# smartroboticslab/okvis2

Measured on AMD Instinct MI355X. Metric: front-end stereo-frames/s (detect+describe+match), 752x480 stereo, higher is better.
Workload: dtype u8/int32 (detect, describe, Hamming) + f64 (match gate); 1 GPU; EuRoC-shaped 752x480 stereo, euroc.yaml front-end params (radius 38, thr 150, <=700 kpts, match thr 60); lanes_per_gpu=1, score_kernels_serialised_across_lanes=False, stereo_frames_per_launch=3072, distinct_frames=256, content=corners, feed=device, cameras_per_multiframe=2, parallelism=frames sharded over 1 GPU(s), no collective

## Files before the change

okvis2_amd/csrc/k_harris.hip:

```cpp
#include <cstdlib>
#include <type_traits>

#include "okvfe_internal.h"

namespace okvfe {

namespace {

constexpr int kTH = 32;
#ifndef OKVFE_K1_WPB
#define OKVFE_K1_WPB 4
#endif
constexpr int kWavesPerBlock = OKVFE_K1_WPB;

__device__ __forceinline__ int mul24(int a, int b) {
  int d;
  asm("v_mul_i32_i24 %0, %1, %2" : "=v"(d) : "v"(a), "v"(b));
  return d;
}
__device__ __forceinline__ int mad24(int a, int b, int c) {
  int d;
  asm("v_mad_i32_i24 %0, %1, %2, %3" : "=v"(d) : "v"(a), "v"(b), "v"(c));
  return d;
}
__device__ __forceinline__ int mad24_10(int a, int c) {
  int d;
  asm("v_mad_i32_i24 %0, %1, 10, %2" : "=v"(d) : "v"(a), "v"(c));
  return d;
}
__device__ __forceinline__ int mul24_3(int a) {
  int d;
  asm("v_mul_i32_i24 %0, 3, %1" : "=v"(d) : "v"(a));
  return d;
}

template <bool ALIGNED>
__device__ __forceinline__ void load_raw(const uint8_t* __restrict__ img, int w, int h, int row,
                                         int x0, int dl, int dc, int dr, uint32_t raw[3]) {
  row = row < 0 ? 0 : (row > h - 1 ? h - 1 : row);
  if (ALIGNED) {
    const uint32_t* rq = reinterpret_cast<const uint32_t*>(img + (size_t)row * (size_t)w);
    raw[0] = rq[dl];
    raw[1] = rq[dc];
    raw[2] = rq[dr];
  } else {
    const uint8_t* rp = img + (size_t)row * (size_t)w;
    uint32_t lo = 0, hi = 0;
#pragma unroll
    for (int i = 0; i < 4; ++i) {
      int c0 = x0 - 2 + i, c1 = x0 + 2 + i;
      c0 = c0 < 0 ? 0 : (c0 > w - 1 ? w - 1 : c0);
      c1 = c1 < 0 ? 0 : (c1 > w - 1 ? w - 1 : c1);
      lo |= (uint32_t)rp[c0] << (8 * i);
      hi |= (uint32_t)rp[c1] << (8 * i);
    }
    raw[0] = lo;
    raw[1] = hi;
    raw[2] = 0;
  }
}

template <bool ALIGNED>
__device__ __forceinline__ void unpack(const uint32_t raw[3], int p[8]) {
  if (ALIGNED) {
    const uint32_t L = raw[0], C = raw[1], R = raw[2];
    p[0] = (L >> 16) & 255;
    p[1] = (L >> 24);
    p[2] = C & 255;
    p[3] = (C >> 8) & 255;
    p[4] = (C >> 16) & 255;
    p[5] = (C >> 24);
    p[6] = R & 255;
    p[7] = (R >> 8) & 255;
  } else {
#pragma unroll
    for (int i = 0; i < 4; ++i) {
      p[i] = (raw[0] >> (8 * i)) & 255;
      p[4 + i] = (raw[1] >> (8 * i)) & 255;
    }
  }
}

__device__ __forceinline__ void cov_row(const int a[8], const int b[8], const int c[8],
                                        const int cmask[6], int rmask, int hs[3][4]) {
  int vs[8], vd[8];
#pragma unroll
  for (int i = 0; i < 8; ++i) {
    vs[i] = mad24_10(b[i], mul24_3(a[i] + c[i]));
    vd[i] = c[i] - a[i];
  }
  int gxx[6], gyy[6], gxy[6];
#pragma unroll
  for (int i = 0; i < 6; ++i) {
    const int m = cmask[i] & rmask;
    const int gx = (vs[i + 2] - vs[i]) & m;
    const int gy = mad24_10(vd[i + 1], mul24_3(vd[i] + vd[i + 2])) & m;
    gxx[i] = mul24(gx, gx) >> 14;
    gyy[i] = mul24(gy, gy) >> 14;
    gxy[i] = mul24(gx, gy) >> 14;
  }
#pragma unroll
  for (int i = 0; i < 4; ++i) {
    hs[0][i] = gxx[i] + 2 * gxx[i + 1] + gxx[i + 2];
    hs[1][i] = gyy[i] + 2 * gyy[i + 1] + gyy[i + 2];
    hs[2][i] = gxy[i] + 2 * gxy[i + 1] + gxy[i + 2];
  }
}

template <bool ALIGNED>
__global__ __launch_bounds__(64 * kWavesPerBlock) void harris_generic_kernel(
    const uint8_t* __restrict__ images, int w, int h, int32_t* __restrict__ scores) {
  const int lane = threadIdx.x;
  const int x0 = (blockIdx.x * 64 + lane) * 4;
  const int wave = __builtin_amdgcn_readfirstlane(threadIdx.y);
  const int ys = (blockIdx.y * kWavesPerBlock + wave) * kTH;
  if (ys >= h || x0 >= w) return;
  const int ye = ys + kTH < h ? ys + kTH : h;
  const size_t img_off = (size_t)blockIdx.z * (size_t)w * (size_t)h;
  const uint8_t* img = images + img_off;
  int32_t* out = scores + img_off + x0;

  const int nd = w >> 2;
  int dc = x0 >> 2;
  dc = dc > nd - 1 ? nd - 1 : dc;
  const int dl = dc > 0 ? dc - 1 : 0;
  const int dr = dc < nd - 1 ? dc + 1 : nd - 1;
  int cmask[6], smask[4];
#pragma unroll
  for (int i = 0; i < 6; ++i) {
    const int col = x0 - 1 + i;
    cmask[i] = (col >= 1 && col <= w - 2) ? -1 : 0;
  }
#pragma unroll
  for (int i = 0; i < 4; ++i) smask[i] = cmask[i + 1];

  int pr[3][8];
  int hsr[3][3][4];
  uint32_t raw[3][3];
  {
    uint32_t t0[3], t1[3];
    load_raw<ALIGNED>(img, w, h, ys - 2, x0, dl, dc, dr, t0);
    load_raw<ALIGNED>(img, w, h, ys - 1, x0, dl, dc, dr, t1);
    load_raw<ALIGNED>(img, w, h, ys, x0, dl, dc, dr, raw[0]);
    load_raw<ALIGNED>(img, w, h, ys + 1, x0, dl, dc, dr, raw[1]);
    unpack<ALIGNED>(t0, pr[0]);
    unpack<ALIGNED>(t1, pr[1]);
  }

  auto step = [&](int j, int s_new, int s_a, int s_b, int h_new, int h_a, int h_b) {
    const int r = ys + j;
    load_raw<ALIGNED>(img, w, h, r + 2, x0, dl, dc, dr, raw[s_new]);
    unpack<ALIGNED>(raw[s_a], pr[s_new]);
    const int g = r - 1;
    const int rmask = (g >= 1 && g <= h - 2) ? -1 : 0;
    cov_row(pr[s_a], pr[s_b], pr[s_new], cmask, rmask, hsr[h_new]);
    const int y = g - 1;
    if (j >= 2 && y < ye) {
      const int ymask = (y >= 1 && y <= h - 2) ? -1 : 0;
      int sc[4];
#pragma unroll
      for (int i = 0; i < 4; ++i) {
        const int A = hsr[h_a][0][i] + 2 * hsr[h_b][0][i] + hsr[h_new][0][i];
        const int B = hsr[h_a][1][i] + 2 * hsr[h_b][1][i] + hsr[h_new][1][i];
        const int Cc = hsr[h_a][2][i] + 2 * hsr[h_b][2][i] + hsr[h_new][2][i];
        const int tq = ((A >> 1) + (B >> 1)) >> 1;
        const int det = mul24(A, B) - mul24(Cc, Cc);
        sc[i] = (det - mul24(tq, tq)) & (smask[i] & ymask);
      }
      int32_t* op = out + (size_t)y * (size_t)w;
      if (ALIGNED) {
        *reinterpret_cast<int4*>(op) = make_int4(sc[0], sc[1], sc[2], sc[3]);
      } else {
#pragma unroll
        for (int i = 0; i < 4; ++i)
          if (x0 + i < w) op[i] = sc[i];
      }
    }
  };

  const int jn = (ye - ys) + 2;
  for (int j = 0; j < jn; j += 3) {
    step(j, 2, 0, 1, 0, 1, 2);
    if (j + 1 < jn) step(j + 1, 0, 1, 2, 1, 2, 0);
    if (j + 2 < jn) step(j + 2, 1, 2, 0, 2, 0, 1);
  }
}


__device__ __forceinline__ int mulhi24(int a, int b) {
  int d;
  asm("v_mul_hi_i32_i24 %0, %1, %2" : "=v"(d) : "v"(a), "v"(b));
  return d;
}
__device__ __forceinline__ void dpp_fence(int& a, int& b, int& c, int& d, int& e, int& f) {
  asm volatile("s_nop 1" : "+v"(a), "+v"(b), "+v"(c), "+v"(d), "+v"(e), "+v"(f));
}
__device__ __forceinline__ void dpp_fence4(int& a, int& b, int& c, int& d) {
  asm volatile("s_nop 1" : "+v"(a), "+v"(b), "+v"(c), "+v"(d));
}
__device__ __forceinline__ void dpp_fence2(int& a, int& b) {
  asm volatile("s_nop 1" : "+v"(a), "+v"(b));
}
__device__ __forceinline__ void lane_neighbours(int a, int b, int& l, int& r) {
  asm("s_nop 1\n\t"
      "v_mov_b32_dpp %0, %2 wave_shr:1 row_mask:0xf bank_mask:0xf bound_ctrl:1\n\t"
      "v_mov_b32_dpp %1, %3 wave_shl:1 row_mask:0xf bank_mask:0xf bound_ctrl:1"
      : "=&v"(l), "=&v"(r)
      : "v"(a), "v"(b));
}
__device__ __forceinline__ int from_left(int v) {
  return __builtin_amdgcn_update_dpp(0, v, 0x138, 0xf, 0xf, true);
}
__device__ __forceinline__ int from_right(int v) {
  return __builtin_amdgcn_update_dpp(0, v, 0x130, 0xf, 0xf, true);
}

constexpr int kStripLanes = 62;
#ifndef OKVFE_K1_WAVES
#define OKVFE_K1_WAVES __attribute__((amdgpu_waves_per_eu(5, 8)))
#endif

struct NmsOut {
  int thr;
  Candidate* cand;
  int cand_cap;
  int32_t* cand_count;
  int32_t* fix_count;
  int32_t* fix_list;
  int no_map;
};

__device__ __forceinline__ int max3i(int a, int b, int c) { return max(max(a, b), c); }
#ifndef OKVFE_K1_SLOTS
#define OKVFE_K1_SLOTS 8
#endif
constexpr int kScoreSlots = OKVFE_K1_SLOTS;
__device__ __forceinline__ void push_hit(uint64_t& mask, uint64_t& ovf, int c, int nb, uint64_t own, uint32_t tag,
                                         uint32_t& sp, uint32_t sp_end) {
  uint64_t sav, pm;
  uint32_t vtag;
  asm volatile(
      "v_cmp_ge_i32_e64 %[mask], %[c], %[nb]\n\t"
      "s_mov_b64 %[ovf], 0\n\t"
      "s_and_b64 %[pm], %[mask], %[own]\n\t"
      "s_cbranch_scc0 .Lokvfe_nopush%=\n\t"
      "s_and_saveexec_b64 %[sav], %[pm]\n\t"
      "v_cmp_gt_u32_e32 vcc, %[end], %[sp]\n\t"
      "s_andn2_b64 %[ovf], exec, vcc\n\t"
      "s_and_b64 exec, exec, vcc\n\t"
      "v_mov_b32 %[vtag], %[tag]\n\t"
      "ds_write2_b32 %[sp], %[c], %[vtag] offset1:64\n\t"
      "v_add_u32 %[sp], %[stride], %[sp]\n\t"
      "s_mov_b64 exec, %[sav]\n"
      ".Lokvfe_nopush%=:"
      : [sp] "+v"(sp), [mask] "=&s"(mask), [ovf] "=&s"(ovf), [sav] "=&s"(sav), [pm] "=&s"(pm), [vtag] "=&v"(vtag)
      : [c] "v"(c), [nb] "v"(nb), [own] "s"(own), [tag] "s"(tag), [end] "s"(sp_end), [stride] "i"(512)
      : "vcc", "scc", "memory");
}

#ifndef OKVFE_K1_STAGE
#define OKVFE_K1_STAGE 248
#endif
constexpr int kCandStage = OKVFE_K1_STAGE;

template <int kTHF, bool NMS, bool PACK = false, bool MEMONLY = false, bool NOMAP = false>
__global__ __launch_bounds__(64 * kWavesPerBlock) OKVFE_K1_WAVES void harris_kernel(
    const uint8_t* __restrict__ images, int w, int h, int32_t* __restrict__ scores, int pitch, int strips,
    int rtiles, int n_images, NmsOut nms, int pack_g, int pack_u, int main_blocks) {
  constexpr int kMain = NMS ? kTHF - 1 : kTHF;
  static_assert(kMain % 6 == 0 && kTHF <= 121, "rows per wave: 6k (+1 with the fused NMS), <= 121");
  constexpr int kSlots = kTHF > 64 ? kScoreSlots + 2 : kScoreSlots;
  const int lane = threadIdx.x;
  const int nd = w >> 2;
  int image, tile, strip, d;
  int sub = 0;
  int group_images = 1;
  bool lane_on = true;
  const bool packed_block = PACK && (int)blockIdx.x >= main_blocks;
  const int wave = __builtin_amdgcn_readfirstlane(threadIdx.y);
  int row_tile;
  if (packed_block) {
    const int p = ((int)blockIdx.x - main_blocks) * kWavesPerBlock + wave;
    const int group = p / rtiles;
    row_tile = p - group * rtiles;
    image = group * pack_g;
    if (image >= n_images) return;
    group_images = n_images - image < pack_g ? n_images - image : pack_g;
    strip = strips;
    sub = lane / pack_u;
    const int j = lane - sub * pack_u;
    lane_on = sub < group_images;
    if (!lane_on) sub = 0;
    d = lane_on ? strip * kStripLanes + j : nd;
  } else {
    const int T = strips * rtiles;
    const int n8 = n_images & ~7;
    const int S = (n8 >> 3) * T;
    const int full = 8 * ((S + kWavesPerBlock - 1) / kWavesPerBlock);
    const int L = (int)blockIdx.x;
    if (L < full) {
      const int s = (L >> 3) * kWavesPerBlock + wave;
      if (s >= S) return;
      const int g = s / T;
      image = g * 8 + (L & 7);
      tile = s - g * T;
    } else {
      const int r = (L - full) * kWavesPerBlock + wave;
      const int i = r / T;
      if (n8 + i >= n_images) return;
      image = n8 + i;
      tile = r - i * T;
    }
    row_tile = tile / strips;
    strip = tile - row_tile * strips;
    d = strip * kStripLanes + lane;
  }
  const int ys_own = row_tile * kTHF;
  if (ys_own >= h) return;
  const int ye_own = ys_own + kTHF < h ? ys_own + kTHF : h;
  const int ys = NMS ? ys_own - 1 : ys_own;
  const bool last_strip = PACK ? packed_block : strip * kStripLanes + 64 >= nd;
  const bool first_lane_halo = packed_block ? d == strip * kStripLanes : (strip != 0 && lane < 1);
  const bool store = d < nd && !first_lane_halo && (last_strip || lane <= kStripLanes);
  const int dcl = d < nd ? d : nd - 1;
  const size_t img_off = (size_t)image * (size_t)w * (size_t)h;
  const __amdgpu_buffer_rsrc_t img_rsrc = __builtin_amdgcn_make_buffer_rsrc(
      const_cast<uint8_t*>(images + img_off), 0, w * h * group_images, 0x00027000);
  const __amdgpu_buffer_rsrc_t out_rsrc = __builtin_amdgcn_make_buffer_rsrc(
      scores + (size_t)image * (size_t)pitch * (size_t)h, 0, pitch * h * 4 * group_images, 0x00027000);
  const int ld_off = dcl * 4 + (PACK ? sub * w * h : 0);
  const bool slotted = NMS && pitch != w;
  const int slot_q = slotted ? d + 2 * strip : d;
  const bool st_on = slotted ? (lane_on && slot_q * 4 < pitch) : store;
  const int st_off = st_on ? slot_q * 16 + (PACK ? sub * pitch * h * 4 : 0) : 0x7FFFFFF0;
  int m0 = d == 0 ? 0 : -1;
  int m3 = d == nd - 1 ? 0 : -1;
  asm volatile("" : "+v"(m0), "+v"(m3));

  auto unpack4 = [](uint32_t c, int p[4]) {
    p[0] = c & 255;
    p[1] = (c >> 8) & 255;
    p[2] = (c >> 16) & 255;
    p[3] = c >> 24;
  };
  (void)unpack4;
  typedef int v4i_t __attribute__((ext_vector_type(4)));
  int win[3][2];
  auto taps = [](int b0, int b1, int b2, int b3) {
    return (int)((uint32_t)(b0 & 255) | ((uint32_t)(b1 & 255) << 8) | ((uint32_t)(b2 & 255) << 16) |
                 ((uint32_t)(b3 & 255) << 24));
  };
  const int r4 = lane & 3;
  int A_above = r4 == 0 ? taps(-24, 0, 24, 0) : r4 == 1 ? taps(0, -24, 0, 24)
              : r4 == 2 ? taps(-24, -80, -24, 0) : taps(0, -24, -80, -24);
  int A_centre = r4 == 0 ? taps(-80, 0, 80, 0) : r4 == 1 ? taps(0, -80, 0, 80) : 0;
  int A_below = r4 == 0 ? taps(-24, 0, 24, 0) : r4 == 1 ? taps(0, -24, 0, 24)
              : r4 == 2 ? taps(24, 80, 24, 0) : taps(0, 24, 80, 24);
  asm volatile("" : "+v"(A_above), "+v"(A_centre), "+v"(A_below));
  auto make_windows = [&](uint32_t dw, int wn[2]) {
    const int x = (int)(dw ^ 0x80808080u);
    int l, r;
    lane_neighbours(x, x, l, r);
    wn[0] = (int)__builtin_amdgcn_alignbyte((uint32_t)x, (uint32_t)l, 3);
    wn[1] = (int)__builtin_amdgcn_alignbyte((uint32_t)r, (uint32_t)x, 1);
  };
  int hs[2][2][4];
  int vp[2][2][4];
#pragma unroll
  for (int q = 0; q < 2; ++q)
#pragma unroll
    for (int c = 0; c < 2; ++c)
#pragma unroll
      for (int i = 0; i < 4; ++i) hs[q][c][i] = vp[q][c][i] = 0;

  int nc[4] = {0, 0, 0, 0}, nh[2][4] = {{0, 0, 0, 0}, {0, 0, 0, 0}}, nl = 0, nr = 0;
  __shared__ int32_t hit_stack[NMS ? kWavesPerBlock * kSlots * 128 : 1];
  constexpr int kStageCap = kCandStage;
  __shared__ Candidate cand_stage[NMS ? kWavesPerBlock : 1][NMS ? kCandStage : 1];
  const uint32_t sp0 = (uint32_t)(uintptr_t)(__attribute__((address_space(3))) int32_t*)hit_stack +
                       (uint32_t)(wave * (kSlots * 512) + lane * 4);
  uint32_t sp = sp0;
  const uint32_t sp_end = (uint32_t)(uintptr_t)(__attribute__((address_space(3))) int32_t*)hit_stack +
                          (uint32_t)((wave + 1) * (kSlots * 512));
  const uint64_t own_lo = __ballot(store && d != 0);
  const uint64_t own_hi = __ballot(store && d != nd - 1);
  const uint64_t real_lanes = __ballot(d < nd);
  const int r_lo = ys_own > 2 ? ys_own : 2;
  const int r_hi = ye_own < h - 2 ? ye_own : h - 2;
  uint64_t rows_adj[2] = {0ull, 0ull};
  auto emit_overflow = [&](uint64_t ovf, int c, int i, int r, bool flag) {
    if ((ovf >> lane) & 1ull) {
      int sub_o = 0;
      if (packed_block) {
        sub_o = lane / pack_u;
        if (sub_o >= group_images) sub_o = 0;
      }
      const int img = image + sub_o;
      const int p = atomicAdd(&nms.cand_count[img], 1);
      if (p < nms.cand_cap) {
        Candidate cd;
        cd.x = dcl * 4 + i;
        cd.y = flag ? r | kCandidateFixupFlag : r;
        cd.score = c;
        nms.cand[(size_t)img * nms.cand_cap + p] = cd;
      }
      if (flag) {
        const int k = atomicAdd(&nms.fix_count[img], 1);
        if (k < kFixListCap) nms.fix_list[(size_t)img * kFixListCap + k] = p;
      }
    }
  };

  auto cov_row = [&](const int* wa, const int* wb, const int* wc, int (*H)[4], bool inner) {
    v4i_t acc1 = {0, 0, 0, 0}, acc2 = {0, 0, 0, 0};
    acc1 = __builtin_amdgcn_mfma_i32_4x4x4i8(A_above, wa[0], acc1, 0, 0, 0);
    acc2 = __builtin_amdgcn_mfma_i32_4x4x4i8(A_above, wa[1], acc2, 0, 0, 0);
    acc1 = __builtin_amdgcn_mfma_i32_4x4x4i8(A_centre, wb[0], acc1, 0, 0, 0);
    acc2 = __builtin_amdgcn_mfma_i32_4x4x4i8(A_centre, wb[1], acc2, 0, 0, 0);
    acc1 = __builtin_amdgcn_mfma_i32_4x4x4i8(A_below, wc[0], acc1, 0, 0, 0);
    acc2 = __builtin_amdgcn_mfma_i32_4x4x4i8(A_below, wc[1], acc2, 0, 0, 0);
#ifndef OKVFE_K1_MFMA_NOPS
#define OKVFE_K1_MFMA_NOPS 7
#endif
#define OKVFE_STR2(x) #x
#define OKVFE_STR(x) OKVFE_STR2(x)
    asm volatile("s_nop " OKVFE_STR(OKVFE_K1_MFMA_NOPS) : "+v"(acc1), "+v"(acc2));
    asm volatile("" ::"v"(wa[0]), "v"(wa[1]), "v"(wb[0]), "v"(wb[1]), "v"(wc[0]), "v"(wc[1]), "v"(A_above), "v"(A_centre),
                 "v"(A_below));
    if (__builtin_expect(!inner, 0)) {
      asm volatile("" ::: "memory");
      acc1 = v4i_t{0, 0, 0, 0};
      acc2 = v4i_t{0, 0, 0, 0};
    }
    int gx[4], gy[4];
    gx[0] = (acc1[0] << 6) & m0;
    gx[1] = acc1[1] << 6;
    gx[2] = acc2[0] << 6;
    gx[3] = (acc2[1] << 6) & m3;
    gy[0] = (acc1[2] << 6) & m0;
    gy[1] = acc1[3] << 6;
    gy[2] = acc2[2] << 6;
    gy[3] = (acc2[3] << 6) & m3;
    int G[2][4];
#pragma unroll
    for (int i = 0; i < 4; ++i) {
      int g0 = mulhi24(gx[i], gx[i]);
      asm("v_mul_hi_i32_i24_sdwa %0, %1, %1 dst_sel:WORD_1 dst_unused:UNUSED_PRESERVE "
          "src0_sel:DWORD src1_sel:DWORD"
          : "+v"(g0)
          : "v"(gy[i]));
      G[0][i] = g0;
      G[1][i] = mulhi24(gx[i], gy[i]);
    }
    dpp_fence4(G[0][0], G[0][3], G[1][0], G[1][3]);
#pragma unroll
    for (int ch = 0; ch < 2; ++ch) {
      int gl, gr;
      lane_neighbours(G[ch][3], G[ch][0], gl, gr);
      const int pm = gl + G[ch][0];
      const int p0 = G[ch][0] + G[ch][1];
      const int p1 = G[ch][1] + G[ch][2];
      const int p2 = G[ch][2] + G[ch][3];
      const int p3 = G[ch][3] + gr;
      H[ch][0] = pm + p0;
      H[ch][1] = p0 + p1;
      H[ch][2] = p1 + p2;
      H[ch][3] = p2 + p3;
    }
  };
  auto score_row = [&](int (*Vp)[4], int (*V)[4], int sc[4]) {
#pragma unroll
    for (int i = 0; i < 4; ++i) {
      const unsigned AB = (unsigned)(Vp[0][i] + V[0][i]);
      const int Cc = Vp[1][i] + V[1][i];
      const int tq = (int)((((AB >> 1) & 0x7FFFu) + (AB >> 17)) >> 1);
      int ab;
      asm("v_mul_u32_u24_sdwa %0, %1, %1 dst_sel:DWORD dst_unused:UNUSED_PAD src0_sel:WORD_0 "
          "src1_sel:WORD_1"
          : "=v"(ab)
          : "v"(AB));
      sc[i] = ab - mad24(tq, tq, mul24(Cc, Cc));
    }
    sc[0] &= m0;
    sc[3] &= m3;
  };
  const bool store_map = !NOMAP && (MEMONLY || !NMS || nms.no_map == 0);
  auto store_row = [&](const int sc[4], int y) {
    if (!store_map) return;
    typedef int v4i __attribute__((ext_vector_type(4)));
    const v4i v = {sc[0], sc[1], sc[2], sc[3]};
    __builtin_amdgcn_raw_buffer_store_b128(v, out_rsrc, st_off, y * pitch * 4, 0);
#ifndef OKVFE_K1_NO_STORE_NOP
    asm volatile("s_nop 1" ::"v"(v));
#endif
  };
  auto nms_row = [&](const int sc[4], int q, bool test, int r) {
    int l, r2;
    lane_neighbours(sc[3], sc[0], l, r2);
    const int hn[4] = {max3i(l, sc[0], sc[1]), max3i(sc[0], sc[1], sc[2]),
                       max3i(sc[1], sc[2], sc[3]), max3i(sc[2], sc[3], r2)};
#ifndef OKVFE_K1_SKIP
#define OKVFE_K1_SKIP 1
#endif
    if (test && r >= r_lo && r < r_hi &&
        (!OKVFE_K1_SKIP || __builtin_amdgcn_ballot_w64(max(nh[q ^ 1][1], nh[q ^ 1][2]) >= nms.thr) != 0ull)) {
      const int lft[4] = {nl, nc[0], nc[1], nc[2]};
      const int rgt[4] = {nc[1], nc[2], nc[3], nr};
      uint64_t mk[4], ovf[4];
#pragma unroll
      for (int i = 0; i < 4; ++i)
        push_hit(mk[i], ovf[i], nc[i], max3i(max3i(nh[q][i], hn[i], lft[i]), rgt[i], nms.thr), i < 2 ? own_lo : own_hi,
                 (uint32_t)(r << 2 | i), sp, sp_end);
      const uint64_t adj = ((mk[0] & mk[1]) | (mk[1] & mk[2]) | (mk[2] & mk[3]) | (mk[3] & (mk[0] >> 1))) & real_lanes;
      if (adj != 0ull) {
        const int t = r - ys_own;
        if (kTHF <= 64 || t < 64)
          rows_adj[0] |= 1ull << t;
        else
          rows_adj[1] |= 1ull << (t - 64);
      }
      if (__builtin_expect((ovf[0] | ovf[1] | ovf[2] | ovf[3]) != 0ull, 0)) {
#pragma unroll
        for (int i = 0; i < 4; ++i) emit_overflow(ovf[i], nc[i], i, r, adj != 0ull);
      }
    }
#pragma unroll
    for (int i = 0; i < 4; ++i) {
      nh[q][i] = hn[i];
      nc[i] = sc[i];
    }
    nl = l;
    nr = r2;
  };

#ifndef OKVFE_K1_AHEAD
#define OKVFE_K1_AHEAD 3
#endif
  constexpr int kAhead = OKVFE_K1_AHEAD;
  static_assert(kAhead >= 1 && kAhead <= 5, "prefetch distance");
  int row_next = ys - 2;
  auto load_next = [&]() -> uint32_t {
    const int r = row_next < 0 ? 0 : (row_next > h - 1 ? h - 1 : row_next);
    ++row_next;
    return (uint32_t)__builtin_amdgcn_raw_buffer_load_b32(img_rsrc, ld_off, r * w, 0);
  };
  uint32_t ring[6];
  {
    const uint32_t t0 = load_next(), t1 = load_next();
#pragma unroll
    for (int i = 0; i < kAhead; ++i) ring[i] = load_next();
    make_windows(t0, win[0]);
    make_windows(t1, win[1]);
  }
  int y = ys - 2;
  auto step = [&](auto ph, auto want_score, auto want_store, auto want_test) {
    constexpr int PH = decltype(ph)::value;
    constexpr int s_new = (PH + 2) % 3, s_a = PH % 3, s_b = (PH + 1) % 3, q = PH % 2;
    ring[(PH + kAhead) % 6] = load_next();
    const int g = y + 1;
    const bool inner = g >= 1 && g <= h - 2;
    if constexpr (MEMONLY) {
      int sc[4];
      unpack4(ring[PH], sc);
      if (decltype(want_store)::value && y < h) store_row(sc, y);
      ++y;
      (void)inner;
      return;
    }
    make_windows(ring[PH], win[s_new]);
    cov_row(win[s_a], win[s_b], win[s_new], hs[q], inner);
#pragma unroll
    for (int ch = 0; ch < 2; ++ch)
#pragma unroll
      for (int i = 0; i < 4; ++i) vp[q][ch][i] = hs[q ^ 1][ch][i] + hs[q][ch][i];
    if (decltype(want_score)::value) {
      int sc[4];
      score_row(vp[q ^ 1], vp[q], sc);
      if (decltype(want_store)::value) {
        if (y < h) store_row(sc, y);
      }
      if (NMS) nms_row(sc, q, decltype(want_test)::value, y - 1);
    }
    ++y;
  };
  using T = std::true_type;
  using F = std::false_type;
#define OKVFE_PH(n) std::integral_constant<int, (n) % 6>()
  step(OKVFE_PH(0), F(), F(), F());
  step(OKVFE_PH(1), F(), F(), F());
  if (NMS) {
    step(OKVFE_PH(2), T(), F(), F());
    step(OKVFE_PH(3), T(), T(), F());
    for (int g = 0; g < kMain / 6; ++g) {
      step(OKVFE_PH(4), T(), T(), T());
      step(OKVFE_PH(5), T(), T(), T());
      step(OKVFE_PH(6), T(), T(), T());
      step(OKVFE_PH(7), T(), T(), T());
      step(OKVFE_PH(8), T(), T(), T());
      step(OKVFE_PH(9), T(), T(), T());
    }
    step(OKVFE_PH(kTHF + 3), T(), F(), T());
  } else {
    for (int g = 0; g < kMain / 6; ++g) {
      step(OKVFE_PH(2), T(), T(), F());
      step(OKVFE_PH(3), T(), T(), F());
      step(OKVFE_PH(4), T(), T(), F());
      step(OKVFE_PH(5), T(), T(), F());
      step(OKVFE_PH(6), T(), T(), F());
      step(OKVFE_PH(7), T(), T(), F());
    }
  }
#undef OKVFE_PH
  if (ys_own == 0 || ye_own == h) {
    const int zero[4] = {0, 0, 0, 0};
    if (ys_own == 0) store_row(zero, 0);
    if (ye_own == h) store_row(zero, h - 1);
  }

  if (NMS) {
    const int cnt = (int)((sp - sp0) >> 9);
    if (!__any(cnt != 0)) return;
    int sub_e = 0;
    if (packed_block) {
      int l2 = lane;
      asm volatile("" : "+v"(l2));
      sub_e = l2 / pack_u;
      if (sub_e >= group_images) sub_e = 0;
    }
    const int image_l = image + sub_e;
    const int x0 = dcl * 4;
    Candidate* outc = nms.cand + (size_t)image_l * nms.cand_cap;
    const int32_t* mine = hit_stack + wave * (kSlots * 128) + lane;
    auto flag_record = [&](int at) {
      const int k = atomicAdd(&nms.fix_count[image_l], 1);
      if (k < kFixListCap) nms.fix_list[(size_t)image_l * kFixListCap + k] = at;
    };
    auto record = [&](int e, bool* flagged) {
      Candidate cd;
      const int tag = mine[e * 128 + 64];
      cd.score = mine[e * 128];
      cd.x = x0 + (tag & 3);
      cd.y = tag >> 2;
      const int t = cd.y - ys_own;
      const uint64_t bit = (kTHF <= 64 || t < 64) ? rows_adj[0] >> t : rows_adj[1] >> (t - 64);
      *flagged = (bit & 1ull) != 0ull;
      if (*flagged) cd.y |= kCandidateFixupFlag;
      return cd;
    };
    auto scan = [&](int c, int* total) {
      int incl = c;
#pragma unroll
      for (int dd = 1; dd < 64; dd <<= 1) {
        const int t = __shfl_up(incl, dd);
        if (lane >= dd) incl += t;
      }
      *total = __builtin_amdgcn_readlane(incl, 63);
      return incl - c;
    };
    if (packed_block) {
      int pos = 0;
      for (int g = 0; g < group_images; ++g) {
        const bool in_g = sub_e == g;
        if (!__any(in_g && cnt != 0)) continue;
        int total;
        const int first = scan(in_g ? cnt : 0, &total);
        int base = 0;
        if (lane == 0) base = atomicAdd(&nms.cand_count[image + g], total);
        base = __builtin_amdgcn_readlane(base, 0);
        if (in_g) pos = base + first;
      }
      for (int e = 0; __any(e < cnt); ++e)
        if (e < cnt) {
          bool fl;
          const Candidate cd = record(e, &fl);
          if (pos + e < nms.cand_cap) outc[pos + e] = cd;
          if (fl) flag_record(pos + e);
        }
    } else {
      int total;
      const int first = scan(cnt, &total);
      int base_l0 = 0;
      if (lane == 0) base_l0 = atomicAdd(&nms.cand_count[image], total);
      constexpr int cap_stage = kStageCap;
      Candidate* stage = cand_stage[wave];
      for (int e = 0; __any(e < cnt); ++e)
        if (e < cnt) {
          bool fl;
          const Candidate cd = record(e, &fl);
          const int idx = first + e;
          if (idx < cap_stage) {
            stage[idx] = cd;
          } else {
            const int at = __builtin_amdgcn_readlane(base_l0, 0) + idx;
            if (at < nms.cand_cap) outc[at] = cd;
          }
          if (fl) flag_record(__builtin_amdgcn_readlane(base_l0, 0) + idx);
        }
      __builtin_amdgcn_wave_barrier();
      const int base = __builtin_amdgcn_readlane(base_l0, 0);
      const int n_staged = total < cap_stage ? total : cap_stage;
      for (int r = lane; r < n_staged; r += 64)
        if (base + r < nms.cand_cap) outc[base + r] = stage[r];
    }
  }
}

}

static int harris_strips(int w) {
  const int nd = w >> 2;
  int strips = 1;
  while ((strips - 1) * kStripLanes + 64 < nd) ++strips;
  return strips;
}

ScoreLayout harris_nms_layout(int w, int h) {
  (void)h;
  static const bool off = lab_env("OKVFE_NO_FUSED_NMS") != nullptr;
  if (off || w % 4 != 0) return ScoreLayout{w, 0};
  const int strips = harris_strips(w);
  if (strips == 1) return ScoreLayout{w, 1};
  const int pitch = ((w + 8 * (strips - 1)) + 31) & ~31;
  return ScoreLayout{pitch, strips};
}

static bool launch_harris_impl(const uint8_t* img, int w, int h, int n_images, int32_t* score,
                               ScoreLayout layout, const NmsOut* nms, hipStream_t stream, bool byte_mover = false) {
  if (n_images <= 0) return true;
  const dim3 block(64, kWavesPerBlock, 1);
  const bool aligned = (w % 4 == 0) && ((reinterpret_cast<uintptr_t>(img) & 3) == 0) &&
                       ((reinterpret_cast<uintptr_t>(score) & 15) == 0);
  if (aligned) {
    const int nd = w >> 2;
    const int strips = harris_strips(w);
    if (nms && !(layout.strips == strips || (layout.strips == 1 && layout.pitch == w))) return false;
    static const int th_env = [] {
      const char* e = lab_env("OKVFE_K1_TH");
      return e ? atoi(e) : 0;
    }();
    const int last_first = (strips - 1) * kStripLanes;
    const int pack_u = nd - last_first;
    const int pack_g = strips >= 2 ? 64 / pack_u : 1;
#define OKVFE_K1_TILING(TH)                                                                     \
  const int rtiles = (h + TH - 1) / TH;   \
  auto main_blocks_of = [&](int nstrips) {                                                       \
    const int T = nstrips * rtiles, n8 = n_images & ~7;                                          \
    return 8 * (((n8 >> 3) * T + kWavesPerBlock - 1) / kWavesPerBlock) +                         \
           ((n_images - n8) * T + kWavesPerBlock - 1) / kWavesPerBlock;                          \
  };
#define OKVFE_K1_NMS_LAUNCH_M(TH, MEM)                                                          \
  {                                                                                              \
    OKVFE_K1_TILING(TH)                                                                          \
    if (pack_g >= 2 && !no_pack) {                                                               \
      const int main_blocks = main_blocks_of(strips - 1);                                        \
      const int groups = (n_images + pack_g - 1) / pack_g;                                       \
      const int pblocks = (groups * rtiles + kWavesPerBlock - 1) / kWavesPerBlock;               \
      if (!MEM && nms->no_map && !generic_nomap)                                                 \
        hipLaunchKernelGGL((harris_kernel<TH, true, true, MEM, !MEM>), dim3(main_blocks + pblocks), \
                           block, 0, stream, img, w, h, score, layout.pitch, strips - 1, rtiles, n_images, *nms, \
                           pack_g, pack_u, main_blocks);                                         \
      else                                                                                       \
      hipLaunchKernelGGL((harris_kernel<TH, true, true, MEM>), dim3(main_blocks + pblocks),      \
                         block, 0, stream, img, w, h, score, layout.pitch, strips - 1, rtiles, n_images, *nms, \
                         pack_g, pack_u, main_blocks);                                           \
    } else {                                                                                     \
      if (!MEM && nms->no_map && !generic_nomap)                                                 \
        hipLaunchKernelGGL((harris_kernel<TH, true, false, MEM, !MEM>), dim3(main_blocks_of(strips)), block, 0, \
                           stream, img, w, h, score, layout.pitch, strips, rtiles, n_images, *nms, 1, 64, 0);  \
      else                                                                                       \
      hipLaunchKernelGGL((harris_kernel<TH, true, false, MEM>), dim3(main_blocks_of(strips)), block, 0,  \
                         stream, img, w, h, score, layout.pitch, strips, rtiles, n_images, *nms, 1, 64, 0);    \
    }                                                                                            \
  }
#define OKVFE_K1_NMS_LAUNCH(TH) OKVFE_K1_NMS_LAUNCH_M(TH, false)
    static const bool no_pack = lab_env("OKVFE_K1_NOPACK") != nullptr;
    static const bool generic_nomap = lab_env("OKVFE_K1_GENERIC_NOMAP") != nullptr;
    if (nms && byte_mover) {
      OKVFE_K1_NMS_LAUNCH_M(61, true);
    } else if (nms) {
      int th = th_env;
      if (th == 0) {
        const int blocks61 = (int)(((long long)strips * ((h + 60) / 61) * n_images + kWavesPerBlock - 1) / kWavesPerBlock);
        th = blocks61 <= 128 ? 25 : 61;
      }
      switch (th) {
        case 25: OKVFE_K1_NMS_LAUNCH(25); break;
#ifdef OKVFE_LAB
        case 31: OKVFE_K1_NMS_LAUNCH(31); break;
        case 37: OKVFE_K1_NMS_LAUNCH(37); break;
        case 43: OKVFE_K1_NMS_LAUNCH(43); break;
        case 49: OKVFE_K1_NMS_LAUNCH(49); break;
        case 55: OKVFE_K1_NMS_LAUNCH(55); break;
        case 91: OKVFE_K1_NMS_LAUNCH(91); break;
        case 121: OKVFE_K1_NMS_LAUNCH(121); break;
#endif
        default: OKVFE_K1_NMS_LAUNCH(61); break;
      }
    } else {
      OKVFE_K1_TILING(30)
      hipLaunchKernelGGL((harris_kernel<30, false>), dim3(main_blocks_of(strips)), block, 0, stream,
                         img, w, h, score, w, strips, rtiles, n_images, NmsOut{}, 1, 64, 0);
    }
#undef OKVFE_K1_NMS_LAUNCH
#undef OKVFE_K1_NMS_LAUNCH_M
#undef OKVFE_K1_TILING
  } else {
    if (nms) return false;
    const dim3 grid((w + 255) / 256, (h + kTH * kWavesPerBlock - 1) / (kTH * kWavesPerBlock),
                    n_images);
    hipLaunchKernelGGL(harris_generic_kernel<false>, grid, block, 0, stream, img, w, h, score);
  }
  return true;
}

void launch_harris(const uint8_t* img, int w, int h, int n_images, int32_t* score,
                   hipStream_t stream) {
  (void)launch_harris_impl(img, w, h, n_images, score, ScoreLayout{w, 0}, nullptr, stream);
}

bool launch_harris_nms(const uint8_t* img, int w, int h, int n_images, int32_t* score,
                       ScoreLayout layout, int abs_threshold, Candidate* cand, int cand_cap,
                       int32_t* cand_count, int32_t* fix_count, int32_t* fix_list, hipStream_t stream,
                       bool store_map) {
  if (layout.strips < 1) return false;
  const NmsOut nms{abs_threshold, cand, cand_cap, cand_count, fix_count, fix_list, store_map ? 0 : 1};
  return launch_harris_impl(img, w, h, n_images, score, layout, &nms, stream);
}

bool launch_harris_byte_mover(const uint8_t* img, int w, int h, int n_images, int32_t* score,
                              ScoreLayout layout, hipStream_t stream) {
  if (layout.strips < 1) return false;
  const NmsOut nms{1, nullptr, 0, nullptr, nullptr, nullptr, 0};
  return launch_harris_impl(img, w, h, n_images, score, layout, &nms, stream, true);
}

}
```

Before: 809,100 stereo-frames/s.

## Add tall 121-row Harris tile path with direct candidate writes for large batches

Adds a tile planner that picks 121-row Harris tiles when the batch is map-free, not packed, and large enough to fill the device for several rounds, and when that reduces total row steps including halo. For the tall variant, the LDS candidate staging buffer is removed and candidates are written straight to global memory using ballot/mbcnt offsets, and the hit-stack slot count is raised. The intent is to cut halo-row recomputation per image and LDS pressure. The cost is fewer, longer waves and possibly lower occupancy.

```diff
diff --git a/okvis2_amd/csrc/harris_tile_plan.h b/okvis2_amd/csrc/harris_tile_plan.h
--- /dev/null
+++ b/okvis2_amd/csrc/harris_tile_plan.h
@@ -0,0 +1,35 @@
+#pragma once
+
+namespace okvfe {
+
+constexpr int kHarrisStripLanes = 62;
+constexpr int kHarrisWavesPerBlock = 4;
+constexpr int kHarrisSmallBlocks = 128;
+constexpr int kHarrisTallMinRounds = 7;
+constexpr int kHarrisTileHeights[] = {25, 61, 121};
+
+inline int harris_strips(int w) {
+  const int nd = w >> 2;
+  int strips = 1;
+  while ((strips - 1) * kHarrisStripLanes + 64 < nd) ++strips;
+  return strips;
+}
+
+inline int harris_tile_steps(int h, int th) { return ((h + th - 1) / th) * (th + 4); }
+
+inline long long harris_tile_waves(int w, int h, int n_images, int th) {
+  return (long long)harris_strips(w) * ((h + th - 1) / th) * n_images;
+}
+
+inline int harris_tile_rows(int w, int h, int n_images, bool map_free, bool packed_last_strip, int wave_slots) {
+  const long long blocks61 = (harris_tile_waves(w, h, n_images, 61) + kHarrisWavesPerBlock - 1) / kHarrisWavesPerBlock;
+  if (blocks61 <= kHarrisSmallBlocks) return 25;
+  int best = 61;
+  if (map_free && !packed_last_strip &&
+      harris_tile_waves(w, h, n_images, 121) >= (long long)kHarrisTallMinRounds * wave_slots &&
+      harris_tile_steps(h, 121) < harris_tile_steps(h, best))
+    best = 121;
+  return best;
+}
+
+}
diff --git a/okvis2_amd/csrc/k_harris.hip b/okvis2_amd/csrc/k_harris.hip
--- a/okvis2_amd/csrc/k_harris.hip
+++ b/okvis2_amd/csrc/k_harris.hip
@@ -1,6 +1,7 @@
 #include <cstdlib>
 #include <type_traits>
 
+#include "harris_tile_plan.h"
 #include "okvfe_internal.h"
 
 namespace okvfe {
@@ -12,6 +13,7 @@
 #define OKVFE_K1_WPB 4
 #endif
 constexpr int kWavesPerBlock = OKVFE_K1_WPB;
+static_assert(kWavesPerBlock == kHarrisWavesPerBlock, "harris_tile_plan.h counts blocks of this many waves");
 
 __device__ __forceinline__ int mul24(int a, int b) {
   int d;
@@ -215,7 +217,7 @@
   return __builtin_amdgcn_update_dpp(0, v, 0x130, 0xf, 0xf, true);
 }
 
-constexpr int kStripLanes = 62;
+constexpr int kStripLanes = kHarrisStripLanes;
 #ifndef OKVFE_K1_WAVES
 #define OKVFE_K1_WAVES __attribute__((amdgpu_waves_per_eu(5, 8)))
 #endif
@@ -235,6 +237,9 @@
 #define OKVFE_K1_SLOTS 8
 #endif
 constexpr int kScoreSlots = OKVFE_K1_SLOTS;
+#ifndef OKVFE_K1_SLOTS_TALL
+#define OKVFE_K1_SLOTS_TALL 15
+#endif
 __device__ __forceinline__ void push_hit(uint64_t& mask, uint64_t& ovf, int c, int nb, uint64_t own, uint32_t tag,
                                          uint32_t& sp, uint32_t sp_end) {
   uint64_t sav, pm;
@@ -269,7 +274,8 @@
     int rtiles, int n_images, NmsOut nms, int pack_g, int pack_u, int main_blocks) {
   constexpr int kMain = NMS ? kTHF - 1 : kTHF;
   static_assert(kMain % 6 == 0 && kTHF <= 121, "rows per wave: 6k (+1 with the fused NMS), <= 121");
-  constexpr int kSlots = kTHF > 64 ? kScoreSlots + 2 : kScoreSlots;
+  constexpr bool kTall = kTHF > 64;
+  constexpr int kSlots = kTall ? OKVFE_K1_SLOTS_TALL : kScoreSlots;
   const int lane = threadIdx.x;
   const int nd = w >> 2;
   int image, tile, strip, d;
@@ -376,7 +382,7 @@
   int nc[4] = {0, 0, 0, 0}, nh[2][4] = {{0, 0, 0, 0}, {0, 0, 0, 0}}, nl = 0, nr = 0;
   __shared__ int32_t hit_stack[NMS ? kWavesPerBlock * kSlots * 128 : 1];
   constexpr int kStageCap = kCandStage;
-  __shared__ Candidate cand_stage[NMS ? kWavesPerBlock : 1][NMS ? kCandStage : 1];
+  __shared__ Candidate cand_stage[NMS ? kWavesPerBlock : 1][NMS && !kTall ? kCandStage : 1];
   const uint32_t sp0 = (uint32_t)(uintptr_t)(__attribute__((address_space(3))) int32_t*)hit_stack +
                        (uint32_t)(wave * (kSlots * 512) + lane * 4);
   uint32_t sp = sp0;
@@ -677,41 +683,54 @@
           if (fl) flag_record(pos + e);
         }
     } else {
-      int total;
-      const int first = scan(cnt, &total);
-      int base_l0 = 0;
-      if (lane == 0) base_l0 = atomicAdd(&nms.cand_count[image], total);
-      constexpr int cap_stage = kStageCap;
-      Candidate* stage = cand_stage[wave];
-      for (int e = 0; __any(e < cnt); ++e)
-        if (e < cnt) {
-          bool fl;
-          const Candidate cd = record(e, &fl);
-          const int idx = first + e;
-          if (idx < cap_stage) {
-            stage[idx] = cd;
-          } else {
-            const int at = __builtin_amdgcn_readlane(base_l0, 0) + idx;
+      if constexpr (kTall) {
+        int total = 0;
+        for (int e = 0; e < kSlots; ++e) total += __popcll(__ballot(e < cnt));
+        int base_l0 = 0;
+        if (lane == 0) base_l0 = atomicAdd(&nms.cand_count[image], total);
+        int at0 = __builtin_amdgcn_readlane(base_l0, 0);
+        for (int e = 0; e < kSlots; ++e) {
+          const uint64_t m = __ballot(e < cnt);
+          if (m == 0ull) break;
+          if (e < cnt) {
+            bool fl;
+            const Candidate cd = record(e, &fl);
+            const int at = at0 + (int)__builtin_amdgcn_mbcnt_hi((uint32_t)(m >> 32), __builtin_amdgcn_mbcnt_lo((uint32_t)m, 0u));
             if (at < nms.cand_cap) outc[at] = cd;
+            if (fl) flag_record(at);
           }
-          if (fl) flag_record(__builtin_amdgcn_readlane(base_l0, 0) + idx);
+          at0 += __popcll(m);
         }
-      __builtin_amdgcn_wave_barrier();
-      const int base = __builtin_amdgcn_readlane(base_l0, 0);
-      const int n_staged = total < cap_stage ? total : cap_stage;
-      for (int r = lane; r < n_staged; r += 64)
-        if (base + r < nms.cand_cap) outc[base + r] = stage[r];
-    }
-  }
-}
-
-}
-
-static int harris_strips(int w) {
-  const int nd = w >> 2;
-  int strips = 1;
-  while ((strips - 1) * kStripLanes + 64 < nd) ++strips;
-  return strips;
+      } else {
+        int total;
+        const int first = scan(cnt, &total);
+        int base_l0 = 0;
+        if (lane == 0) base_l0 = atomicAdd(&nms.cand_count[image], total);
+        constexpr int cap_stage = kStageCap;
+        Candidate* stage = cand_stage[wave];
+        for (int e = 0; __any(e < cnt); ++e)
+          if (e < cnt) {
+            bool fl;
+            const Candidate cd = record(e, &fl);
+            const int idx = first + e;
+            if (idx < cap_stage) {
+              stage[idx] = cd;
+            } else {
+              const int at = __builtin_amdgcn_readlane(base_l0, 0) + idx;
+              if (at < nms.cand_cap) outc[at] = cd;
+            }
+            if (fl) flag_record(__builtin_amdgcn_readlane(base_l0, 0) + idx);
+          }
+        __builtin_amdgcn_wave_barrier();
+        const int base = __builtin_amdgcn_readlane(base_l0, 0);
+        const int n_staged = total < cap_stage ? total : cap_stage;
+        for (int r = lane; r < n_staged; r += 64)
+          if (base + r < nms.cand_cap) outc[base + r] = stage[r];
+      }
+    }
+  }
+}
+
 }
 
 ScoreLayout harris_nms_layout(int w, int h) {
@@ -778,13 +797,25 @@
     if (nms && byte_mover) {
       OKVFE_K1_NMS_LAUNCH_M(61, true);
     } else if (nms) {
+      static const int wave_slots = [] {
+        int dev = 0, cus = 0;
+        if (hipGetDevice(&dev) != hipSuccess ||
+            hipDeviceGetAttribute(&cus, hipDeviceAttributeMultiprocessorCount, dev) != hipSuccess || cus <= 0)
+          cus = 256;
+        return cus * 4 * 5;
+      }();
       int th = th_env;
-      if (th == 0) {
-        const int blocks61 = (int)(((long long)strips * ((h + 60) / 61) * n_images + kWavesPerBlock - 1) / kWavesPerBlock);
-        th = blocks61 <= 128 ? 25 : 61;
-      }
+      if (th == 0)
+        th = harris_tile_rows(w, h, n_images, nms->no_map && !generic_nomap, pack_g >= 2 && !no_pack, wave_slots);
       switch (th) {
         case 25: OKVFE_K1_NMS_LAUNCH(25); break;
+#ifndef OKVFE_LAB
+        case 121: {
+          OKVFE_K1_TILING(121)
+          hipLaunchKernelGGL((harris_kernel<121, true, false, false, true>), dim3(main_blocks_of(strips)), block, 0,
+                             stream, img, w, h, score, layout.pitch, strips, rtiles, n_images, *nms, 1, 64, 0);
+        } break;
+#endif
 #ifdef OKVFE_LAB
         case 31: OKVFE_K1_NMS_LAUNCH(31); break;
         case 37: OKVFE_K1_NMS_LAUNCH(37); break;
```

Result: no change. 813,300 stereo-frames/s (median of 6 runs) (+0.5%).
